# okieraised/rs-face-detection-tflite

Measured on AMD Instinct MI355X. Metric: faces/sec at batch=256 (256x256 back-camera) per GPU, higher is better.
Workload: dtype f32

## Files before the change

rs-face-detection-tflite_amd/csrc/engine.cpp:

```cpp
#include "engine.hpp"
#include "launch.hpp"

#include <algorithm>
#include <cstdio>
#include <cstdlib>
#include <cstring>
#include <stdexcept>

namespace mi {

void hip_check(hipError_t e, const char* what) {
    if (e != hipSuccess) throw std::runtime_error(std::string(what) + ": " + hipGetErrorString(e));
}

namespace {
template <class T>
void upload(T*& dev, std::vector<T>& host, const char* what_alloc, const char* what_copy) {
    if (dev) hip_check(hipFree(dev), "hipFree");
    dev = nullptr;
    if (host.empty()) return;
    hip_check(hipMalloc(reinterpret_cast<void**>(&dev), host.size() * sizeof(T)), what_alloc);
    hip_check(hipMemcpy(dev, host.data(), host.size() * sizeof(T), hipMemcpyHostToDevice), what_copy);
    std::vector<T>().swap(host);
}
// ... 24 lines not shown
    if (d_in_stage_) hipFree(d_in_stage_);
    free_bandnet();
    for (float* p : d_out_)
        if (p) hipFree(p);
    for (hipStream_t st : side_streams_) hipStreamDestroy(st);
    for (hipEvent_t ev : lane_events_) hipEventDestroy(ev);
    for (hipStream_t st : head_streams_) hipStreamDestroy(st);
    for (hipEvent_t ev : head_events_) if (ev) hipEventDestroy(ev);
    if (stream_) hipStreamDestroy(stream_);
}

void Model::invalidate_graphs() {
    if (!graphs_.empty()) (void)hipDeviceSynchronize();
    for (auto& kv : graphs_) hipGraphExecDestroy(kv.second);
    graphs_.clear();
}

struct Model::Option {
    enum { kReplan = 1,
           kFreeSmall = 2,
           kKeepGraphs = 4,
           kOneOf = 8,
           kKiB = 16 , kWriteOnly = 32, kReadOnly = 64,
           kBandGen = 128,
           kForms = 256 };
    const char* key;
    int Model::*field;
    int lo, hi, flags;
};

const Model::Option* Model::find_option(const std::string& key) {
    using O = Option;
    constexpr int kMax = 0x7fffffff;
    static const Option table[] = {
        {"chunk", &Model::chunk_, 0, kMax, 0},
        {"graph", &Model::use_graph_, 0, 1, 0},
        {"fuse", &Model::fuse_level_, 0, 5, O::kReplan},
        {"res_budget", &Model::res_budget_, 16, 156, O::kReplan | O::kKiB},
        {"pipe", &Model::pipe_max_, 0, 4, O::kReplan},
        {"small_chain", &Model::small_chain_, 0, 64, O::kFreeSmall},
        {"pipe_rows", &Model::pipe_rows_, 1 << 1 | 1 << 2 | 1 << 4, 0, O::kOneOf},
        {"pipe_band", &Model::pipe_band_, 0, 4096, 0},
        {"strip", &Model::strip_, 0, 1, 0},
        {"stem_fuse", &Model::stem_fuse_, 0, 1, 0},
        {"stem_mfma", &Model::stem_mfma_, 0, 2, O::kForms},
        {"conv_mfma", &Model::conv_mfma_, 0, 1, 0},
        {"conv_bf16", &Model::conv_bf16_, 0, 2, O::kReplan},
        {"stem_run", &Model::stem_run_, 0, 32, 0},
        {"pair_fuse", &Model::pair_fuse_, 0, 1, 0},
        {"mdb_band", &Model::mdb_band_, 0, 4096, 0},
        {"chain_fixed", &Model::chain_fixed_, 0, 1, 0},
        {"chain_sched", &Model::chain_sched_, 0, 1, 0},
        {"mchain", &Model::mchain_, 0, 1, 0},
        {"tail", &Model::tail_, 0, 1, O::kReplan},
        {"tail_pre", &Model::tail_pre_, 0, 2, 0},
        {"tail_g", &Model::tail_g_, 0, 64, 0},
        {"band", &Model::band_, 0, 2, O::kReplan},
        {"band_test_fail", &Model::band_test_fail_, 0, 1, O::kWriteOnly},
        {"band_test_absent", &Model::band_test_absent_, 0, 256, O::kWriteOnly},
        {"band_test_gen", nullptr, 0, kMax, O::kBandGen | O::kWriteOnly},
        {"band_wide", &Model::band_wide_ok_, 0, 1, O::kReplan},
        {"band_fork", &Model::band_fork_, 0, 1, O::kReplan},
        {"band_nw", &Model::band_nw_, 8, 256, O::kReplan},
        {"band_fail_streak", &Model::band_fail_streak_, 0, 0, O::kReadOnly},
        {"band_wraps", &Model::band_wraps_, 0, 0, O::kReadOnly},
        {"fork", &Model::fork_, 0, 1, 0},
        {"heads", &Model::head_streams_opt_, 1, kHeadStreams, O::kReplan},
        {"reuse", &Model::reuse_, 0, 1, O::kReplan},
        {"lanes", &Model::lanes_, 1, 4, 0},
        {"test_poison", &Model::test_poison_, 1 << 1 | 1 << 2, 0, O::kOneOf | O::kKeepGraphs},
    };
    for (const Option& o : table)
        if (key == o.key) return &o;
    return nullptr;
}

void Model::set_option(const std::string& key, int value) {
    const Option* o = find_option(key);
    if (!o || (o->flags & Option::kReadOnly)) throw std::runtime_error("unknown option '" + key + "'");
    int v = (o->lo == 0 && o->hi == 1) ? value != 0 : std::min(o->hi, std::max(o->lo, value));
    if (o->flags & Option::kOneOf) v = (value >= 0 && value < 31 && (o->lo >> value & 1)) ? value : 0;
    if (o->flags & Option::kForms) v = (value >= o->lo && value <= o->hi) ? value : 1;
    if (o->flags & Option::kKiB) v *= 1024;
    if (o->flags & Option::kBandGen) { band_gen_ = static_cast<unsigned>(v); band_gen_force_ = true; }
    else this->*o->field = v;
    if (o->flags & Option::kKeepGraphs) return;
    if (o->flags & Option::kReplan) dirty_ = true;
    if ((o->flags & Option::kFreeSmall) && d_small_) { hipFree(d_small_); d_small_ = nullptr; small_floats_ = 0; }
    invalidate_graphs();
    chunk_cap_ = 0;
}

int Model::get_option(const std::string& key) const {
    const Option* o = find_option(key);
    if (!o || (o->flags & Option::kWriteOnly)) throw std::runtime_error("unknown option '" + key + "'");
    const int v = this->*o->field;
    return (o->flags & Option::kKiB) ? v / 1024 : v;
}

void Model::rebuild() {
    if (d_small_) { hipFree(d_small_); d_small_ = nullptr; small_floats_ = 0; }
    hip_check(hipSetDevice(device_), "hipSetDevice");
    invalidate_graphs();
    plan_ = build_plan(parse_tflite(blob_.data(), blob_.size()), fuse_level_, pipe_max_, res_budget_, tail_ != 0);
    if (!reuse_) {
        long off = 0;
// ... 137 lines not shown
                const int Cm = g.tensors[m.in[0]].shape[3];
                if (m.kind == Node::Conv) macs += elems(m.out) * m.KH * m.KW * Cm * batch;
                else macs += static_cast<double>(mo[1]) * mo[2] * Cm * ((m.w >= 0 ? 9 : 0) + mo[3]) * batch;
                for (int c : {m.w, m.b, m.w2, m.b2, m.alpha}) bytes += 4 * elems(c);
            }
        }
        if (n.kind == Node::Chain) {
            for (int t : n.extra_out) bytes += 4 * elems(t) * batch;
            for (const Node& m : n.members) {
                const auto& mo = g.tensors[m.out].shape;
                macs += static_cast<double>(mo[1]) * mo[2] * g.tensors[m.in[0]].shape[3] * (9 + mo[3]) * batch;
            }
            for (const Node& m : n.members)
                for (int c : {m.w, m.b, m.w2, m.b2, m.alpha}) bytes += 4 * elems(c);
            for (const Node& m : n.head_nodes) {
                macs += elems(m.out) * g.tensors[m.in[0]].shape[3] * batch;
                for (int c : {m.w, m.b, m.w2, m.b2}) bytes += 4 * elems(c);
            }
        }
        st.bytes += bytes;
        st.macs += macs;
        auto dims = [](const std::vector<int>& sh) {
            std::string d;
            for (size_t q = 1; q < sh.size(); q++) d += (q > 1 ? "x" : "") + std::to_string(sh[q]);
            return d;
        };
        if (static_cast<int>(i) == first.launches[k].node) st.detail = dims(si) + "->";
        st.detail = st.detail.substr(0, st.detail.find("->") + 2) + dims(so);
    }
    return stats;
}

LaunchCtx Model::launch_ctx(const float* in, int chunk_start, int frames) const {
    LaunchCtx c;
    c.weights = d_weights_;
    c.arena = d_arena_ + static_cast<size_t>(plan_.arena_floats_per_frame) * chunk_cap_ * arena_lane_;
    c.in = in; c.out = d_out_.data();
    c.small = d_small_; c.small_floats = small_floats_;
    c.progs = d_programs_; c.tail_progs = d_tail_programs_;
    c.band_prog = d_band_prog_; c.band_consts = d_band_consts_; c.band_ws = d_band_ws_; c.band_sync = d_band_sync_; c.band_fail = d_band_fail_;
    c.chunk_cap = chunk_cap_; c.chunk_start = chunk_start; c.F = frames;
    c.u8_frames = u8_.frames; c.u8_lut = u8_.lut; c.u8_frame_bytes = u8_.frame_bytes; c.u8_row_bytes = u8_.row_bytes;
    c.strip = strip_; c.pair_fuse = pair_fuse_; c.stem_fuse = stem_fuse_; c.stem_mfma = stem_mfma_; c.stem_run = stem_run_; c.mchain = mchain_; c.conv_mfma = conv_mfma_; c.conv_bf16 = conv_bf16_;
    c.small_chain = small_chain_; c.lanes = lanes_;
    c.pipe_rows = pipe_rows_; c.pipe_band = pipe_band_; c.mdb_band = mdb_band_; c.tail_pre = tail_pre_; c.tail_g = tail_g_;
    c.fork = fork_ && lanes_ == 1;
    c.cu_count = device_cu_count();
    c.band = band_use_ && chunk_start == 0;
    c.band_test_absent = band_test_absent_;
    return c;
}

namespace {
int issue(const Launch& l, hipStream_t s, int chain_fixed, int chain_sched) {
    auto many = [&](int (*f)(const BlockArgs*, int, void*)) { return f(l.blocks.data(), static_cast<int>(l.blocks.size()), s); };
    switch (l.to) {
        case Launcher::Conv: return launch_conv(std::get<ConvArgs>(l.args), s);
        case Launcher::HeadGemm: return launch_head_gemm(std::get<HeadGemmArgs>(l.args), s);
        case Launcher::Dw: return launch_dw(std::get<DwArgs>(l.args), s);
        case Launcher::Xc: return launch_xc(std::get<XcArgs>(l.args), s);
        case Launcher::Mdblock: return launch_mdblock(std::get<DblockArgs>(l.args), s);
        case Launcher::Dblock: return launch_dblock(std::get<DblockArgs>(l.args), s);
        case Launcher::Mbneck: return launch_mbneck(std::get<BneckArgs>(l.args), s);
        case Launcher::Bneck: return launch_bneck(std::get<BneckArgs>(l.args), s);
        case Launcher::Tail: return launch_tail(std::get<TailLaunch>(l.args), s);
        case Launcher::Resident: return launch_resident(std::get<ResLaunch>(l.args), s);
        case Launcher::Chain: return launch_chain(std::get<ChainArgs>(l.args), s, chain_fixed, chain_sched);
        case Launcher::StripPipe: return many(launch_strip_pipe);
        case Launcher::MstripChain: return many(launch_mstrip_chain);
        case Launcher::SmallChain: {
            int rc = 0;
            for (size_t k = 0; k < l.blocks.size() && rc == 0; k++) rc = l.blocks[k].sh == 1 ? launch_strip(l.blocks[k], s) : launch_block(l.blocks[k], s);
            return rc;
        }
        case Launcher::Ms2: return launch_ms2(std::get<BlockArgs>(l.args), s);
        case Launcher::Mwalk: return launch_mwalk(std::get<BlockArgs>(l.args), s);
        case Launcher::Strip: return launch_strip(std::get<BlockArgs>(l.args), s);
        case Launcher::Mstrip: return launch_mstrip(std::get<BlockArgs>(l.args), s);
        case Launcher::Block: return launch_block(std::get<BlockArgs>(l.args), s);
        case Launcher::Add: return launch_add(std::get<EltArgs>(l.args), s);
        case Launcher::Act: return launch_act(std::get<EltArgs>(l.args), s);
        case Launcher::Maxpool: return launch_maxpool(std::get<EltArgs>(l.args), s);
        case Launcher::Padc: return launch_padc(std::get<EltArgs>(l.args), s);
        case Launcher::Resize2x: return launch_resize2x(std::get<EltArgs>(l.args), s);
        case Launcher::DepthToSpace: return launch_depth_to_space(std::get<EltArgs>(l.args), s);
        case Launcher::Bandnet: return launch_bandnet(std::get<BandLaunch>(l.args), s);
        case Launcher::Avgpool: return launch_avgpool(std::get<EltArgs>(l.args), s);
        case Launcher::L2norm: return launch_l2norm_rows(std::get<EltArgs>(l.args), s);
        case Launcher::Transpose: return launch_transpose(std::get<EltArgs>(l.args), s);
    }
    return 0;
}
}

void Model::enqueue_chunk(const float* in, int chunk_start, int F, hipStream_t trunk, std::vector<hipEvent_t>* marks, Lowered* keep) {
    LaunchCtx ctx = launch_ctx(in, chunk_start, F);
    if (marks) ctx.fork = false;
    Lowered low = lower_chunk(plan_, consts_, band_plan_, sched_, ctx, keep != nullptr);
    auto mark = [&] {
        if (!marks) return;
        hipEvent_t ev;
        hip_check(hipEventCreate(&ev), "hipEventCreate");
        hip_check(hipEventRecord(ev, trunk), "hipEventRecord");
        marks->push_back(ev);
    };
    mark();
    const size_t n_launches = low.launches.size(), start_event = plan_.nodes.size();
    auto event = [&](size_t k) {
        if (head_events_.size() < plan_.nodes.size() + 2 + kHeadStreams) head_events_.resize(plan_.nodes.size() + 2 + kHeadStreams, nullptr);
        if (!head_events_[k]) hip_check(hipEventCreateWithFlags(&head_events_[k], hipEventDisableTiming), "hipEventCreate");
        return head_events_[k];
    };
    unsigned used_heads = 0;
    for (size_t k = 0; k < n_launches; k++) {
        const Launch& l = low.launches[k];
        hipStream_t s = trunk;
        if (l.slot >= 0) {
            while (static_cast<int>(head_streams_.size()) <= l.slot) {
                hipStream_t st;
                hip_check(hipStreamCreateWithFlags(&st, hipStreamNonBlocking), "hipStreamCreate");
                head_streams_.push_back(st);
            }
            s = head_streams_[static_cast<size_t>(l.slot)];
            if (l.wait >= 0) {
                hip_check(wait_event(s, event(static_cast<size_t>(low.launch_of_node[static_cast<size_t>(l.wait)]))), "hipStreamWaitEvent");
            } else {
                hip_check(record_event(event(start_event), trunk), "hipEventRecord");
                hip_check(wait_event(s, event(start_event)), "hipStreamWaitEvent");
            }
            used_heads |= 1u << l.slot;
        }
        int rc = 0;
        for (int rep = 0; rep < (marks ? profile_inner_ : 1) && rc == 0; rep++) rc = issue(l, s, chain_fixed_, chain_sched_);
        if (rc != 0) throw std::runtime_error(std::string("kernel launch failed: ") + hipGetErrorString(static_cast<hipError_t>(rc)));
        if (l.record) hip_check(record_event(event(k), s), "hipEventRecord");
        mark();
    }
    for (int k = 0; k < kHeadStreams; k++)
        if (used_heads & (1u << k)) {
            hip_check(record_event(event(start_event + 1 + static_cast<size_t>(k)), head_streams_[static_cast<size_t>(k)]), "hipEventRecord");
            hip_check(wait_event(trunk, event(start_event + 1 + static_cast<size_t>(k))), "hipStreamWaitEvent");
        }
    last_chunk_frames_ = F;
    if (keep) *keep = std::move(low);
}

void Model::enqueue_all(const float* in, int batch, hipStream_t s) {
    if (lanes_ > 1 && batch > chunk_cap_) {
        while (static_cast<int>(side_streams_.size()) < lanes_ - 1) {
            hipStream_t st;
            hip_check(hipStreamCreateWithFlags(&st, hipStreamNonBlocking), "hipStreamCreate");
            side_streams_.push_back(st);
        }
        while (static_cast<int>(lane_events_.size()) < lanes_) {
            hipEvent_t ev;
            hip_check(hipEventCreateWithFlags(&ev, hipEventDisableTiming), "hipEventCreate");
            lane_events_.push_back(ev);
        }
        hip_check(record_event(lane_events_[0], s), "hipEventRecord");
        int lane = 0;
        for (int start = 0; start < batch; start += chunk_cap_, lane = (lane + 1) % lanes_) {
            hipStream_t ls = lane == 0 ? s : side_streams_[lane - 1];
            if (lane > 0 && start < chunk_cap_ * lanes_) hip_check(wait_event(ls, lane_events_[0]), "hipStreamWaitEvent");
            arena_lane_ = lane;
            enqueue_chunk(in, start, std::min(chunk_cap_, batch - start), ls);
        }
        arena_lane_ = 0;
        for (int l = 1; l < lanes_; l++) {
            hip_check(record_event(lane_events_[l], side_streams_[l - 1]), "hipEventRecord");
            hip_check(wait_event(s, lane_events_[l]), "hipStreamWaitEvent");
        }
        return;
    }
    int chunk = chunk_cap_;
    for (int start = 0; start < batch; start += chunk) enqueue_chunk(in, start, std::min(chunk, batch - start), s);
}

bool Model::takes_u8_input() {
    if (dirty_) rebuild();
    return mi::takes_u8_input(plan_, consts_);
}

void Model::poison_scratch(hipStream_t s) {
    const int byte = test_poison_ == 1 ? 0xFF : 0x7F;
    if (d_arena_) hip_check(hipMemsetAsync(d_arena_, byte, std::max<size_t>(arena_floats_, 64) * sizeof(float), s), "hipMemsetAsync poison arena");
    if (d_small_) hip_check(hipMemsetAsync(d_small_, byte, small_floats_ * sizeof(float), s), "hipMemsetAsync poison small-batch scratch");
// ... 167 lines not shown
```

rs-face-detection-tflite_amd/csrc/engine.hpp:

```cpp
#pragma once

#include <hip/hip_runtime.h>

#include <map>
#include <memory>
#include <string>
#include <vector>

#include "bandplan.hpp"
#include "consts.hpp"
#include "launches.hpp"
#include "plan.hpp"

namespace mi {

void hip_check(hipError_t e, const char* what);

class Model {
   public:
    Model(const uint8_t* bytes, size_t n, int device);
    ~Model();
    Model(const Model&) = delete;
    Model& operator=(const Model&) = delete;

    int device() const { return device_; }
    const Graph& graph() const { return plan_.graph; }
    const Plan& plan() const { return plan_; }
    std::vector<int> input_dims() const { return plan_.graph.tensors[plan_.graph.inputs[0]].shape; }
    int num_outputs() const { return static_cast<int>(plan_.graph.outputs.size()); }
    const std::vector<int>& output_dims(int i) const { return plan_.graph.tensors[plan_.graph.outputs.at(i)].shape; }
    size_t output_elems(int i) const { return plan_.graph.tensors[plan_.graph.outputs.at(i)].elems(); }
    size_t input_elems() const { return plan_.graph.tensors[plan_.graph.inputs[0]].elems(); }

    void run_device(const float* in, int batch, hipStream_t stream, bool one_shot = false);
    bool band_failed();
    int get_option(const std::string& key) const;
    int band_workgroups(int batch);
    void run(const float* in, int batch, float* const* outs, int mem, hipStream_t stream);
    float* output_device(int i) const { return d_out_.at(i); }
    hipStream_t stream() const { return stream_; }
    bool takes_u8_input();
    void run_device_u8(const uint8_t* frames, long frame_bytes, int row_bytes, const float* lut, int batch, hipStream_t stream);

    struct LaunchStat {
        std::string kernel, detail;
        double ms = 0, bytes = 0, macs = 0;
    };
    std::vector<LaunchStat> profile(const float* in, int batch, int reps, hipStream_t stream);
    void set_option(const std::string& key, int value);
    size_t debug_tensor(int tensor, int frame, float* dst, size_t cap);
    std::string describe() const { return plan_.describe(); }

   private:
    void rebuild();
    struct Option;
    static const Option* find_option(const std::string& key);
    void build_bandnet();
    void free_bandnet();
    bool band_usable(int batch) const;
    void band_before_launch(hipStream_t s);
    void poison_scratch(hipStream_t s);
    void ensure_capacity(int batch);
    LaunchCtx launch_ctx(const float* in, int chunk_start, int frames) const;
    void enqueue_chunk(const float* in, int chunk_start, int frames, hipStream_t s, std::vector<hipEvent_t>* marks = nullptr, Lowered* keep = nullptr);
    void enqueue_all(const float* in, int batch, hipStream_t s);
    void invalidate_graphs();

    int device_ = 0;
    std::vector<uint8_t> blob_;
    Plan plan_;
    int fuse_level_ = 5, pipe_max_ = 4, tail_ = 1, reuse_ = 1;
    int res_budget_ = 156 * 1024;
    int chunk_ = 0, lanes_ = 1, use_graph_ = 1;
    int fork_ = 1, head_streams_opt_ = 1;
    int conv_mfma_ = 1;
    int conv_bf16_ = 0;
    int strip_ = 1, stem_fuse_ = 1, stem_mfma_ = 1, stem_run_ = 0, pair_fuse_ = 1, mchain_ = 1, chain_fixed_ = 1, chain_sched_ = 1;
    int pipe_rows_ = 0, pipe_band_ = 0, mdb_band_ = 0;
    int tail_pre_ = 0, tail_g_ = 0;
    int arena_lane_ = 0;
    std::vector<hipStream_t> side_streams_;
    std::vector<hipEvent_t> lane_events_;
    SideSchedule sched_;
    std::vector<hipStream_t> head_streams_;
    std::vector<hipEvent_t> head_events_;
    bool dirty_ = true;

    float* d_weights_ = nullptr;
    PlanConsts consts_;
    int profile_inner_ = 1;

    ResStage* d_programs_ = nullptr;
    TailStage* d_tail_programs_ = nullptr;
    float* d_arena_ = nullptr;
    size_t arena_floats_ = 0;
    int chunk_cap_ = 0;
    int batch_cap_ = 0;
    std::vector<float*> d_out_;
    float* d_in_stage_ = nullptr;
    size_t in_stage_floats_ = 0;
    int last_chunk_frames_ = 0;

    int band_ = 1;
    int band_nw_ = 128;
    BandPlan band_plan_;
    bool band_use_ = false;
    bool band_ran_ = false;
    int band_test_fail_ = 0;
    int band_test_absent_ = 0;
    int test_poison_ = 0;
    int band_fail_streak_ = 0;
    bool band_disabled_ = false;
    unsigned band_gen_ = 0;
    bool band_gen_force_ = false;
    int band_wraps_ = 0;
    size_t band_ws_bytes_ = 0;
    int band_fork_ = 1, band_wide_ok_ = 1;
    BandPacked* d_band_prog_ = nullptr;
    float* d_band_consts_ = nullptr;
    float* d_band_ws_ = nullptr;
    unsigned* d_band_sync_ = nullptr;
    int* h_band_fail_ = nullptr;
    int* d_band_fail_ = nullptr;

    hipStream_t stream_ = nullptr;
    int small_chain_ = 16;
    float* d_small_ = nullptr;
    size_t small_floats_ = 0;
    struct GraphKey {
        const void* in;
// ... 24 lines not shown
```

rs-face-detection-tflite_amd/csrc/kernels.hpp:

```cpp
#pragma once

#include <cstddef>
#include <cstdint>

namespace mi {

enum ActKind : int { ACT_NONE = 0, ACT_RELU = 1, ACT_RELU6 = 2, ACT_PRELU = 3 };
enum ResMode : int { RES_NONE = 0, RES_DIRECT = 1, RES_MAXPOOL = 2, RES_UP2X = 3 };

struct Epilogue {
    const float* bias = nullptr;
    const float* alpha = nullptr;
    const float* res = nullptr;
    long res_fs = 0;
    int res_mode = RES_NONE;
    int res_C = 0;
    int res_W = 0, res_H = 0;
    int act = ACT_NONE;
    int res_after = 0;
};

struct ConvArgs {
    const float* in = nullptr;
    const uint8_t* in_u8 = nullptr;
// ... 223 lines not shown
    unsigned mHWp = 0, mWp = 0;
    long w_a = -1;
    long w_c = -1;
};
struct TailLaunch {
    const TailStage* prog = nullptr;
    int nstages = 0, B = 0;
    int G = 1;
    int frame_floats = 0;
    int variant = 0;
    ResBases bases;
};
int launch_tail(const TailLaunch& a, void* stream);
bool tail_stage_ok(int kind, int K, int S, int src_C, int Kv, int Co, bool dst_lds);
unsigned tail_magic(int d);

int launch_conv(const ConvArgs& a, void* stream);
const char* conv_kernel_label(const ConvArgs& a);
bool conv_takes_u8(const ConvArgs& a);
bool conv_mfma_shape_ok(int C, int KH, int KW, int Co);
bool conv_mfma_supports(const ConvArgs& a);
int launch_conv_mfma(const ConvArgs& a, void* stream);
bool conv_bf16_supports(const ConvArgs& a);
int launch_conv_bf16(const ConvArgs& a, void* stream);
int launch_dw(const DwArgs& a, void* stream);
int launch_block(const BlockArgs& a, void* stream);
bool block_kernel_supports(const BlockArgs& a);
const char* block_kernel_label(const BlockArgs& a, char* buf, size_t cap);
int launch_strip(const BlockArgs& a, void* stream);
bool strip_kernel_supports(const BlockArgs& a);
bool strip_shape_ok(int C, int Co);
int strip_consts_floats(int C);
void strip_pack_consts(int C, const float* w_dw, const float* b_dw, const float* w_pw, const float* bias, const float* alpha, int act, float* dst);
const char* strip_kernel_label(const BlockArgs& a, char* buf, size_t cap);
int launch_mwalk(const BlockArgs& a, void* stream);
bool mwalk_kernel_supports(const BlockArgs& a);
bool mwalk_shape_ok(int W, int C, int Co);
int mwalk_consts_floats(int W, int C, int Co);
void mwalk_pack_consts(int W, int C, int Co, const float* w_dw, const float* b_dw, const float* w_pw, const float* bias, const float* alpha, int act, float* dst);
const char* mwalk_kernel_label(const BlockArgs& a, char* buf, size_t cap);
int launch_ms2(const BlockArgs& a, void* stream);
bool ms2_kernel_supports(const BlockArgs& a);
bool ms2_shape_ok(int W, int C, int Co, bool skip);
int ms2_consts_floats(int W, int C, int Co, bool skip);
void ms2_pack_consts(int W, int C, int Co, bool skip, const float* w_dw, const float* b_dw, const float* w_pw, const float* bias, const float* alpha, int act, float* dst);
const char* ms2_kernel_label(const BlockArgs& a, char* buf, size_t cap);
int launch_mstrip(const BlockArgs& a, void* stream);
bool mstrip_kernel_supports(const BlockArgs& a);
bool mstrip_shape_ok(int C, int Co);
int mstrip_consts_floats(int C);
void mstrip_pack_consts(int C, const float* w_dw, const float* b_dw, const float* w_pw, const float* bias, const float* alpha, int act, float* dst);
const char* mstrip_kernel_label(const BlockArgs& a, char* buf, size_t cap);
bool mstrip_chain_supports(const BlockArgs* blocks, int n);
int launch_mstrip_chain(const BlockArgs* blocks, int n, void* stream);
bool strip_pipe_supports(const BlockArgs* blocks, int n);
bool strip_pipe_shape_ok(int C, int W);
bool strip_tail_shape_ok(int C, int Co, int H, int W);
int strip_consts_s2_floats(int C, int Co);
void strip_pack_consts_s2(int C, int Co, const float* w_dw, const float* b_dw, const float* w_pw, const float* bias, const float* alpha, int act, float* dst);
int launch_strip_pipe(const BlockArgs* blocks, int n, void* stream);
const char* strip_pipe_label(const BlockArgs* blocks, int n, char* buf, size_t cap);
int strip_pipe_rows_per_step(int H, int hint = 0);
int launch_chain(const ChainArgs& a, void* stream, int fixed = 1, int sched = 1);

struct BneckBlock {
    const float* w1 = nullptr;
    const float* w2 = nullptr;
    const float* consts = nullptr;
    float hi1 = 0.f, hi2 = 0.f;
    const float* mconsts = nullptr;
    int act1 = ACT_RELU, act2 = ACT_RELU;
};
constexpr int kMaxBneck = 6;
struct BneckArgs {
    const float* in = nullptr;
    float* out = nullptr;
    long in_fs = 0, out_fs = 0;
    int B = 0, H = 0, W = 0, C = 0, Cm = 0, nblocks = 0;
    int bands = 1;
    BneckBlock blocks[kMaxBneck];
};
struct XcStage {
    const float* cblob = nullptr;
    int has_dw = 1;
    const float* w_pw = nullptr;
    int C = 0, Co = 0;
    int act = ACT_RELU;
    int skip = 0;
    const float* res = nullptr;
    long res_fs = 0;
    int res_C = 0, res_W = 0;
};
constexpr int kMaxXc = 8;
struct XcArgs {
    const float* in = nullptr;
    float* out = nullptr;
    long in_fs = 0, out_fs = 0;
    int B = 0, H = 0, W = 0, nstages = 0;
    XcStage st[kMaxXc];
};
bool xc_kernel_supports(const XcArgs& a);
int xc_const_floats(int C, int Co);
int launch_xc(const XcArgs& a, void* stream);
struct DblockArgs {
    const float* in = nullptr;
    float* out = nullptr;
    long in_fs = 0, out_fs = 0;
// ... 133 lines not shown
```

rs-face-detection-tflite_amd/csrc/mstrip_kernels.hip:

```cpp
#include <hip/hip_runtime.h>

#include <algorithm>
#include <cstdint>
#include <cstdio>
#include <cstdlib>
#include <type_traits>
#include <utility>

#include "kernels.hpp"
#include "launch.hpp"
#include "mrow.hpp"

namespace mi {

namespace {

struct MstripArgs {
    const float* in;
    float* out;
    const float* consts;
    long in_fs, out_fs;
    int B, H;
    int bands, band_rows;
    int has_res;
    float hi;
    unsigned long long* stamps;
};

constexpr int kMstripChain = 8;
struct MstripChainArgs {
    const float* in[kMstripChain];
    float* out[kMstripChain];
    const float* consts[kMstripChain];
    long in_fs[kMstripChain], out_fs[kMstripChain];
    int has_res[kMstripChain];
    float hi[kMstripChain];
    int nblocks, B, H;
};

template <int CK>
struct MK {
    static constexpr int C = 4 * CK, MT = C / 16;
    static constexpr int QP = CK + 1;
    static constexpr int PS = 4 * QP;
    static constexpr int IMG_F = 34 * PS;
    static constexpr int DPX = 64 / QP;
    static constexpr int NLD = 32 / DPX;
    static_assert(32 % DPX == 0 && NLD == 8, "eight DMA instructions per row (two source bases, four immediate offsets each)");
    static_assert((16 * PS) % 64 == 0 && 16 * PS / 64 < 256, "ds_read2st64_b32 reaches the second pixel tile");
    static constexpr int OFF_A = 0, A_F = CK * MT * 64, OFF_TAP = A_F, TAP_F = CK * 48, OFF_BIAS = OFF_TAP + TAP_F, OFF_SLOPE = OFF_BIAS + C, TOTAL = OFF_SLOPE + C;
    static constexpr int WG_F = A_F + 2 * C + TAP_F;
    static constexpr int NBUF = 2;
};

#ifdef MI_MSTRIP_STAMPS
struct MstripStamps { unsigned long long acc[7] = {0, 0, 0, 0, 0, 0, 0}, prev = __builtin_amdgcn_s_memtime(); };
#define MI_MSTAMP(k) { __builtin_amdgcn_sched_barrier(0); unsigned long long t_ = __builtin_amdgcn_s_memtime(); asm volatile("s_waitcnt lgkmcnt(0)" ::: "memory"); st.acc[k] += t_ - st.prev; st.prev = t_; __builtin_amdgcn_sched_barrier(0); }
#else
struct MstripStamps {};
#define MI_MSTAMP(k)
#endif

template <int CK>
__device__ __forceinline__ void mstrip_issue_row(const float* in, const int r, const int H, const unsigned lds_img, const int bi, const int goff) {
    using K = MK<CK>;
    mrow_dma2<K::C, K::PS, K::DPX, K::DPX * K::QP>(reinterpret_cast<const char*>(in + (long)min(max(r, 0), H - 1) * 32 * K::C),
                                                   lds_img + (unsigned)((bi * K::IMG_F + K::PS) * 4), goff);
}

template <int CK, bool RELU, class HR>
__device__ __forceinline__ void mstrip_walk(const float* in, float* out, const float* wgc, float* img, const unsigned lds_img, const int goff, const HR has_res,
                                            const float hi, const int H, const int y0, const int y1, const int lane, MstripStamps& st) {
    using K = MK<CK>;
    constexpr int C = K::C, MT = K::MT, PS = K::PS, QP = K::QP, IMG_F = K::IMG_F, NLD = K::NLD;
    const int kq = lane >> 4, p = lane & 15;
    float tap[CK][9];
    mrow_load_taps9<CK>(reinterpret_cast<const float4*>(wgc + K::A_F + 2 * C) + kq * 3, tap);
    MI_MSTAMP(0)
    typedef __attribute__((address_space(3))) float lfloat;
    const unsigned x_lds = (unsigned)(uintptr_t)(lfloat*)(img + p * PS + kq);
    const unsigned a_lds = (unsigned)(uintptr_t)(lfloat*)const_cast<float*>(wgc + lane);
    const float* sme = img + (1 + p) * PS + 4 * kq;
    const unsigned ooff = (unsigned)(p * C + 4 * kq) * 4u;

    float accA[CK][2], accB[CK][2];
    df32x4 D[MT][2];
#pragma unroll
    for (int ks = 0; ks < CK; ks++) accA[ks][0] = accA[ks][1] = accB[ks][0] = accB[ks][1] = 0.f;

    constexpr int NST = 2 * MT;
    auto step = [&](auto emit, int r, float (&aPN)[CK][2], float (&aC)[CK][2]) {
        const int t = r - (y0 - 1), bi = t & 1;
        mrow_wait<NST, NLD>(t - 1 >= 2, t == 0 || (t - 1) + 2 <= (y1 - y0 + 1));
        if (r < 0 || r >= H) mrow_clear_row<32 * QP>(img + bi * IMG_F + PS, lane);
        wave_sync();
        MI_MSTAMP(1)
        mstrip_row<CK, MT, PS, decltype(emit)::value>(x_lds + (unsigned)(bi * IMG_F * 4), a_lds, tap, aPN, aC, D);
        MI_MSTAMP(2)
        __builtin_amdgcn_sched_barrier(0);
        if constexpr (decltype(emit)::value) mrow_store_row<RELU, C, 32>(D, (gchar*)(out + (long)(r - 1) * 32 * C), ooff, wgc + K::A_F + C + 4 * kq, hi, p);
        MI_MSTAMP(3)
        __builtin_amdgcn_sched_barrier(0);
        mrow_init_acc<C, PS>(D, wgc + K::A_F + 4 * kq, sme + bi * IMG_F, has_res != 0);
        __builtin_amdgcn_sched_barrier(0);
        wave_sync();
        __builtin_amdgcn_s_waitcnt(0xC07F);
        if (r + 2 <= y1) mstrip_issue_row<CK>(in, r + 2, H, lds_img, bi, goff);
        MI_MSTAMP(4)
    };
    step(std::false_type{}, y0 - 1, accA, accB);
    step(std::false_type{}, y0, accB, accA);
    for (int r = y0 + 1; r <= y1; r += 2) {
        step(std::true_type{}, r, accA, accB);
        if (r + 1 > y1) break;
        step(std::true_type{}, r + 1, accB, accA);
    }
}

template <int CK, bool RELU>
__global__ __launch_bounds__(256, 2) void mstrip_kernel(MstripArgs a) {
    using K = MK<CK>;
    constexpr int C = K::C, PS = K::PS, QP = K::QP, IMG_F = K::IMG_F, NLD = K::NLD, NBUF = K::NBUF;
    extern __shared__ __attribute__((aligned(16))) float lds[];
    MstripStamps st;
    const int lane = threadIdx.x & 63;
    const int wave = __builtin_amdgcn_readfirstlane(threadIdx.x >> 6);
    float* wgc = lds;
    float* img = lds + K::WG_F + wave * NBUF * IMG_F;
    const int unit = blockIdx.x * 4 + wave;
    const int band = unit / a.B, b = unit - band * a.B;
    const bool active = band < a.bands;
    const int y0 = band * a.band_rows, y1 = min(y0 + a.band_rows, a.H);
    const float* in = a.in + (long)b * a.in_fs;
    const int goff = mrow_goff<CK>(lane);
    const unsigned lds_img = __builtin_amdgcn_readfirstlane((unsigned)(uintptr_t)(__attribute__((address_space(3))) float*)img);
    mrow_clear_border<QP, NBUF, IMG_F, 33 * PS>(img, lane);

    if (active) mstrip_issue_row<CK>(in, y0 - 1, a.H, lds_img, 0, goff);
    MI_MSTAMP(5)
    for (int i = threadIdx.x; i < K::A_F / 4; i += 256) reinterpret_cast<float4*>(wgc)[i] = reinterpret_cast<const float4*>(a.consts + K::OFF_A)[i];
    for (int i = threadIdx.x; i < 2 * C; i += 256) wgc[K::A_F + i] = a.consts[K::OFF_BIAS + i];
    for (int i = threadIdx.x; i < K::TAP_F / 4; i += 256) reinterpret_cast<float4*>(wgc + K::A_F + 2 * C)[i] = reinterpret_cast<const float4*>(a.consts + K::OFF_TAP)[i];
    if (active) mstrip_issue_row<CK>(in, y0, a.H, lds_img, 1, goff);
    if (active) wait_vm<NLD>(); else wait_vm<0>();
    MI_MSTAMP(6)
    asm volatile("s_waitcnt lgkmcnt(0)" ::: "memory");
    __builtin_amdgcn_s_barrier();
    asm volatile("" ::: "memory");
    if (!active) return;
    mstrip_walk<CK, RELU>(in, a.out + (long)b * a.out_fs, wgc, img, lds_img, goff, a.has_res != 0, a.hi, a.H, y0, y1, lane, st);
#ifdef MI_MSTRIP_STAMPS
    if (a.stamps && lane == 0)
        for (int k = 0; k < 7; k++) a.stamps[(long)unit * 8 + k] = st.acc[k];
#endif
}

template <int CK, bool RELU>
__global__ __launch_bounds__(512, 2) void mstrip_chain_kernel(MstripChainArgs ca) {
    using K = MK<CK>;
    constexpr int C = K::C, PS = K::PS, QP = K::QP, IMG_F = K::IMG_F, NLD = K::NLD, NBUF = K::NBUF;
    extern __shared__ __attribute__((aligned(16))) float lds[];
    MstripStamps st;
    const int lane = threadIdx.x & 63;
    const int wave = __builtin_amdgcn_readfirstlane(threadIdx.x >> 6);
    float* img = lds + 2 * K::WG_F + wave * NBUF * IMG_F;
    const int b = blockIdx.x;
    const int y0 = 4 * wave, y1 = y0 + 4;
    const int goff = mrow_goff<CK>(lane);
    const unsigned lds_img = __builtin_amdgcn_readfirstlane((unsigned)(uintptr_t)(__attribute__((address_space(3))) float*)img);
    mrow_clear_border<QP, NBUF, IMG_F, 33 * PS>(img, lane);

    for (int i = threadIdx.x; i < K::A_F / 4; i += 512) reinterpret_cast<float4*>(lds)[i] = reinterpret_cast<const float4*>(ca.consts[0] + K::OFF_A)[i];
    for (int i = threadIdx.x; i < 2 * C; i += 512) lds[K::A_F + i] = ca.consts[0][K::OFF_BIAS + i];
    for (int i = threadIdx.x; i < K::TAP_F / 4; i += 512) reinterpret_cast<float4*>(lds + K::A_F + 2 * C)[i] = reinterpret_cast<const float4*>(ca.consts[0] + K::OFF_TAP)[i];
    for (int blk = 0; blk < ca.nblocks; blk++) {
        float* wgc = lds + (blk & 1) * K::WG_F;
        const float* in = ca.in[blk] + (long)b * ca.in_fs[blk];
        const int has_res = ca.has_res[blk];
        const float hi = ca.hi[blk];
        float* const outp = ca.out[blk] + (long)b * ca.out_fs[blk];
        mstrip_issue_row<CK>(in, y0 - 1, ca.H, lds_img, 0, goff);
        constexpr int NPRE = (K::WG_F / 4 + 511) / 512;
        float4 pre[NPRE];
        const bool more = blk + 1 < ca.nblocks;
        if (more) {
            const float* cn = ca.consts[blk + 1];
#pragma unroll
            for (int k = 0; k < NPRE; k++) {
                const int i = threadIdx.x + 512 * k;
                const int src = i < K::A_F / 4 ? K::OFF_A + 4 * i : (i < (K::A_F + 2 * C) / 4 ? K::OFF_BIAS + 4 * i - K::A_F : K::OFF_TAP + 4 * i - K::A_F - 2 * C);
                pre[k] = i < K::WG_F / 4 ? *reinterpret_cast<const float4*>(cn + src) : make_float4(0.f, 0.f, 0.f, 0.f);
            }
        }
        mstrip_issue_row<CK>(in, y0, ca.H, lds_img, 1, goff);
        wait_vm<NLD>();
        asm volatile("s_waitcnt lgkmcnt(0)" ::: "memory");
        if (blk == 0) {
            __builtin_amdgcn_s_barrier();
            asm volatile("" ::: "memory");
        }
        mstrip_walk<CK, RELU>(in, outp, wgc, img, lds_img, goff, has_res, hi, ca.H, y0, y1, lane, st);
        asm volatile("s_waitcnt vmcnt(0)" ::: "memory");
        if (more) {
            float* nx = lds + ((blk + 1) & 1) * K::WG_F;
#pragma unroll
            for (int k = 0; k < NPRE; k++) {
                const int i = threadIdx.x + 512 * k;
                if (i < K::WG_F / 4) reinterpret_cast<float4*>(nx)[i] = pre[k];
            }
        }
        asm volatile("s_waitcnt vmcnt(0) lgkmcnt(0)" ::: "memory");
        __builtin_amdgcn_s_barrier();
        asm volatile("" ::: "memory");
    }
}

}

bool mstrip_shape_ok(int C, int Co) {
    static const bool off = getenv("MI_NO_MSTRIP") != nullptr;
    return !off && C == Co && C == 48;
}

bool mstrip_kernel_supports(const BlockArgs& a) {
    if (!a.w_strip || !a.has_dw || a.sh != 1 || a.sw != 1 || a.pt != 1 || a.pl != 1) return false;
    if (!mstrip_shape_ok(a.C, a.Co) || a.W != 32 || a.H != a.Ho || a.W != a.Wo || a.H < 2) return false;
    if (a.ep.res_mode != RES_NONE) {
        if (a.ep.res_after) return false;
        if (a.ep.res_mode != RES_DIRECT || a.ep.res != a.in || a.ep.res_fs != a.in_fs || a.ep.res_C != a.C) return false;
    }
    static const int min_b = getenv("MI_MSTRIP_MIN_B") ? atoi(getenv("MI_MSTRIP_MIN_B")) : 32;
    if (a.B < min_b) return false;
    auto aligned16 = [](const void* p) { return (reinterpret_cast<uintptr_t>(p) & 15) == 0; };
    return aligned16(a.in) && aligned16(a.out) && !(a.in_fs & 3) && !(a.out_fs & 3);
}

int mstrip_consts_floats(int C) { return C == 48 ? MK<12>::TOTAL : 0; }

void mstrip_pack_consts(int C, const float* w_dw, const float* b_dw, const float* w_pw, const float* bias, const float* alpha, int act, float* dst) {
    using K = MK<12>;
    std::fill(dst, dst + mstrip_consts_floats(C), 0.f);
    mrow_pack_a(dst + K::OFF_A, w_pw, C / 4, K::MT, C);
    mrow_pack_taps(dst + K::OFF_TAP, w_dw, C / 4);
    mrow_pack_bias(dst + K::OFF_BIAS, dst + K::OFF_SLOPE, C, C, w_pw, b_dw, bias, alpha, act);
}

const char* mstrip_kernel_label(const BlockArgs& a, char* buf, size_t cap) {
    snprintf(buf, cap, "mstrip_kernel<%d,%d>", a.C / 4, a.ep.act == ACT_RELU ? 1 : 0);
    return buf;
}

bool mstrip_chain_supports(const BlockArgs* blocks, int n) {
    static const bool off = getenv("MI_NO_MSTRIP_CHAIN") != nullptr;
    if (off || n < 2 || n > kMstripChain) return false;
    for (int k = 0; k < n; k++) {
        const BlockArgs& a = blocks[k];
        if (!mstrip_kernel_supports(a) || a.H != 32 || a.B != blocks[0].B || (a.ep.act == ACT_RELU) != (blocks[0].ep.act == ACT_RELU)) return false;
        if (k && a.in != blocks[k - 1].out) return false;
    }
    return true;
}

int launch_mstrip_chain(const BlockArgs* blocks, int n, void* stream) {
    using K = MK<12>;
    if (!mstrip_chain_supports(blocks, n)) return (int)hipErrorInvalidValue;
    MstripChainArgs ca{};
    ca.nblocks = n; ca.B = blocks[0].B; ca.H = blocks[0].H;
    for (int k = 0; k < n; k++) {
        const BlockArgs& a = blocks[k];
        ca.in[k] = a.in; ca.out[k] = a.out; ca.consts[k] = a.w_strip; ca.in_fs[k] = a.in_fs; ca.out_fs[k] = a.out_fs;
        ca.has_res[k] = a.ep.res_mode == RES_DIRECT;
        ca.hi[k] = a.ep.act == ACT_RELU6 ? 6.f : INFINITY;
    }
    const size_t lds_bytes = (size_t)(2 * K::WG_F + 8 * K::NBUF * K::IMG_F) * 4;
    return mrow_launch(mstrip_chain_kernel<12, true>, mstrip_chain_kernel<12, false>, blocks[0].ep.act == ACT_RELU, dim3((unsigned)ca.B), dim3(512), lds_bytes,
                       (hipStream_t)stream, ca);
}

unsigned long long* g_mstrip_stamps = nullptr;

int launch_mstrip(const BlockArgs& a, void* stream) {
    using K = MK<12>;
    MstripArgs ma;
    ma.stamps = g_mstrip_stamps;
    ma.in = a.in; ma.out = a.out; ma.consts = a.w_strip; ma.in_fs = a.in_fs; ma.out_fs = a.out_fs;
    ma.B = a.B; ma.H = a.H;
    static const int forced = getenv("MI_MSTRIP_BAND") ? atoi(getenv("MI_MSTRIP_BAND")) : 0;
    long bands = std::max<long>(1, (8L * device_cu_count() + a.B / 2) / std::max(1, a.B));
    int rows = (int)((a.H + bands - 1) / bands);
    rows = std::max(rows, std::min(a.H, 4));
    if (forced > 0) rows = std::min(forced, a.H);
    ma.band_rows = rows;
    ma.bands = (a.H + rows - 1) / rows;
    ma.has_res = a.ep.res_mode == RES_DIRECT;
    ma.hi = a.ep.act == ACT_RELU6 ? 6.f : INFINITY;
    const long units = (long)a.B * ma.bands;
    const size_t lds_bytes = (size_t)(K::WG_F + 4 * K::NBUF * K::IMG_F) * 4;
    return mrow_launch(mstrip_kernel<12, true>, mstrip_kernel<12, false>, a.ep.act == ACT_RELU, dim3((unsigned)((units + 3) / 4)), dim3(256), lds_bytes,
                       (hipStream_t)stream, ma);
}

}
```

Measured before the change: 224,700.

## Hand over chained mstrip block boundary rows through LDS instead of refetching

In the multi-block mstrip chain kernel, the last output row of each block is also written into the LDS image buffer, and the next block's first input row is prefetched during the final step. The next block then skips its initial global row fetches and waits. The next block's weights are prefetched with raw asm loads so the vmcnt wait at block end can be dropped. This removes per-block startup latency and global reloads, at the cost of extra barriers and more fragile wait-count reasoning. Optional timestamp instrumentation is added alongside.

```diff
diff --git a/rs-face-detection-tflite_amd/csrc/engine.cpp b/rs-face-detection-tflite_amd/csrc/engine.cpp
--- a/rs-face-detection-tflite_amd/csrc/engine.cpp
+++ b/rs-face-detection-tflite_amd/csrc/engine.cpp
@@ -100,6 +100,7 @@
         {"chain_fixed", &Model::chain_fixed_, 0, 1, 0},
         {"chain_sched", &Model::chain_sched_, 0, 1, 0},
         {"mchain", &Model::mchain_, 0, 1, 0},
+        {"mchain_lds", &Model::mchain_lds_, 0, 1, 0},
         {"tail", &Model::tail_, 0, 1, O::kReplan},
         {"tail_pre", &Model::tail_pre_, 0, 2, 0},
         {"tail_g", &Model::tail_g_, 0, 64, 0},
@@ -343,7 +344,7 @@
 }
 
 namespace {
-int issue(const Launch& l, hipStream_t s, int chain_fixed, int chain_sched) {
+int issue(const Launch& l, hipStream_t s, int chain_fixed, int chain_sched, int mchain_lds) {
     auto many = [&](int (*f)(const BlockArgs*, int, void*)) { return f(l.blocks.data(), static_cast<int>(l.blocks.size()), s); };
     switch (l.to) {
         case Launcher::Conv: return launch_conv(std::get<ConvArgs>(l.args), s);
@@ -358,7 +359,7 @@
         case Launcher::Resident: return launch_resident(std::get<ResLaunch>(l.args), s);
         case Launcher::Chain: return launch_chain(std::get<ChainArgs>(l.args), s, chain_fixed, chain_sched);
         case Launcher::StripPipe: return many(launch_strip_pipe);
-        case Launcher::MstripChain: return many(launch_mstrip_chain);
+        case Launcher::MstripChain: return launch_mstrip_chain(l.blocks.data(), static_cast<int>(l.blocks.size()), s, mchain_lds);
         case Launcher::SmallChain: {
             int rc = 0;
             for (size_t k = 0; k < l.blocks.size() && rc == 0; k++) rc = l.blocks[k].sh == 1 ? launch_strip(l.blocks[k], s) : launch_block(l.blocks[k], s);
@@ -422,7 +423,7 @@
             used_heads |= 1u << l.slot;
         }
         int rc = 0;
-        for (int rep = 0; rep < (marks ? profile_inner_ : 1) && rc == 0; rep++) rc = issue(l, s, chain_fixed_, chain_sched_);
+        for (int rep = 0; rep < (marks ? profile_inner_ : 1) && rc == 0; rep++) rc = issue(l, s, chain_fixed_, chain_sched_, mchain_lds_);
         if (rc != 0) throw std::runtime_error(std::string("kernel launch failed: ") + hipGetErrorString(static_cast<hipError_t>(rc)));
         if (l.record) hip_check(record_event(event(k), s), "hipEventRecord");
         mark();
diff --git a/rs-face-detection-tflite_amd/csrc/engine.hpp b/rs-face-detection-tflite_amd/csrc/engine.hpp
--- a/rs-face-detection-tflite_amd/csrc/engine.hpp
+++ b/rs-face-detection-tflite_amd/csrc/engine.hpp
@@ -75,7 +75,7 @@
     int fork_ = 1, head_streams_opt_ = 1;
     int conv_mfma_ = 1;
     int conv_bf16_ = 0;
-    int strip_ = 1, stem_fuse_ = 1, stem_mfma_ = 1, stem_run_ = 0, pair_fuse_ = 1, mchain_ = 1, chain_fixed_ = 1, chain_sched_ = 1;
+    int strip_ = 1, stem_fuse_ = 1, stem_mfma_ = 1, stem_run_ = 0, pair_fuse_ = 1, mchain_ = 1, mchain_lds_ = 1, chain_fixed_ = 1, chain_sched_ = 1;
     int pipe_rows_ = 0, pipe_band_ = 0, mdb_band_ = 0;
     int tail_pre_ = 0, tail_g_ = 0;
     int arena_lane_ = 0;
diff --git a/rs-face-detection-tflite_amd/csrc/kernels.hpp b/rs-face-detection-tflite_amd/csrc/kernels.hpp
--- a/rs-face-detection-tflite_amd/csrc/kernels.hpp
+++ b/rs-face-detection-tflite_amd/csrc/kernels.hpp
@@ -299,7 +299,7 @@
 void mstrip_pack_consts(int C, const float* w_dw, const float* b_dw, const float* w_pw, const float* bias, const float* alpha, int act, float* dst);
 const char* mstrip_kernel_label(const BlockArgs& a, char* buf, size_t cap);
 bool mstrip_chain_supports(const BlockArgs* blocks, int n);
-int launch_mstrip_chain(const BlockArgs* blocks, int n, void* stream);
+int launch_mstrip_chain(const BlockArgs* blocks, int n, void* stream, int lds_handover = 1);
 bool strip_pipe_supports(const BlockArgs* blocks, int n);
 bool strip_pipe_shape_ok(int C, int W);
 bool strip_tail_shape_ok(int C, int Co, int H, int W);
diff --git a/rs-face-detection-tflite_amd/csrc/mstrip_kernels.hip b/rs-face-detection-tflite_amd/csrc/mstrip_kernels.hip
--- a/rs-face-detection-tflite_amd/csrc/mstrip_kernels.hip
+++ b/rs-face-detection-tflite_amd/csrc/mstrip_kernels.hip
@@ -36,6 +36,9 @@
     int has_res[kMstripChain];
     float hi[kMstripChain];
     int nblocks, B, H;
+#ifdef MI_MSTRIP_STAMPS
+    unsigned long long* stamps;
+#endif
 };
 
 template <int CK>
@@ -53,8 +56,9 @@
     static constexpr int NBUF = 2;
 };
 
-#ifdef MI_MSTRIP_STAMPS
-struct MstripStamps { unsigned long long acc[7] = {0, 0, 0, 0, 0, 0, 0}, prev = __builtin_amdgcn_s_memtime(); };
+constexpr int kMstripStampSlots = 12;
+#ifdef MI_MSTRIP_STAMPS
+struct MstripStamps { unsigned long long acc[kMstripStampSlots] = {0, 0, 0, 0, 0, 0, 0, 0, 0, 0, 0, 0}, prev = __builtin_amdgcn_s_memtime(); };
 #define MI_MSTAMP(k) { __builtin_amdgcn_sched_barrier(0); unsigned long long t_ = __builtin_amdgcn_s_memtime(); asm volatile("s_waitcnt lgkmcnt(0)" ::: "memory"); st.acc[k] += t_ - st.prev; st.prev = t_; __builtin_amdgcn_sched_barrier(0); }
 #else
 struct MstripStamps {};
@@ -68,9 +72,14 @@
                                                    lds_img + (unsigned)((bi * K::IMG_F + K::PS) * 4), goff);
 }
 
-template <int CK, bool RELU, class HR>
+struct MstripHand {
+    bool first, give;
+    const float* next;
+};
+template <int CK, bool RELU, bool HAND = false, class HR>
 __device__ __forceinline__ void mstrip_walk(const float* in, float* out, const float* wgc, float* img, const unsigned lds_img, const int goff, const HR has_res,
-                                            const float hi, const int H, const int y0, const int y1, const int lane, MstripStamps& st) {
+                                            const float hi, const int H, const int y0, const int y1, const int lane, MstripStamps& st,
+                                            const MstripHand hand = MstripHand{true, false, nullptr}) {
     using K = MK<CK>;
     constexpr int C = K::C, MT = K::MT, PS = K::PS, QP = K::QP, IMG_F = K::IMG_F, NLD = K::NLD;
     const int kq = lane >> 4, p = lane & 15;
@@ -91,7 +100,12 @@
     constexpr int NST = 2 * MT;
     auto step = [&](auto emit, int r, float (&aPN)[CK][2], float (&aC)[CK][2]) {
         const int t = r - (y0 - 1), bi = t & 1;
-        mrow_wait<NST, NLD>(t - 1 >= 2, t == 0 || (t - 1) + 2 <= (y1 - y0 + 1));
+        const bool handing = HAND && decltype(emit)::value && hand.next && r == y1;
+        if (handing) {
+            dwg_barrier();
+            MI_MSTAMP(10)
+        }
+        if (!HAND || hand.first || t != 0) mrow_wait<NST, NLD>(t - 1 >= 2, t == 0 || (t - 1) + 2 <= (y1 - y0 + 1));
         if (r < 0 || r >= H) mrow_clear_row<32 * QP>(img + bi * IMG_F + PS, lane);
         wave_sync();
         MI_MSTAMP(1)
@@ -99,6 +113,9 @@
         MI_MSTAMP(2)
         __builtin_amdgcn_sched_barrier(0);
         if constexpr (decltype(emit)::value) mrow_store_row<RELU, C, 32>(D, (gchar*)(out + (long)(r - 1) * 32 * C), ooff, wgc + K::A_F + C + 4 * kq, hi, p);
+        if constexpr (HAND && decltype(emit)::value) {
+            if (handing && hand.give) mrow_store_a<RELU, C, PS>(D, const_cast<float*>(sme) + K::NBUF * IMG_F, wgc + K::A_F + C + 4 * kq, hi, true, kq);
+        }
         MI_MSTAMP(3)
         __builtin_amdgcn_sched_barrier(0);
         mrow_init_acc<C, PS>(D, wgc + K::A_F + 4 * kq, sme + bi * IMG_F, has_res != 0);
@@ -106,6 +123,7 @@
         wave_sync();
         __builtin_amdgcn_s_waitcnt(0xC07F);
         if (r + 2 <= y1) mstrip_issue_row<CK>(in, r + 2, H, lds_img, bi, goff);
+        else if (handing) mstrip_issue_row<CK>(hand.next, y0, H, lds_img, 1, goff);
         MI_MSTAMP(4)
     };
     step(std::false_type{}, y0 - 1, accA, accB);
@@ -155,7 +173,7 @@
 #endif
 }
 
-template <int CK, bool RELU>
+template <int CK, bool RELU, bool LDSH>
 __global__ __launch_bounds__(512, 2) void mstrip_chain_kernel(MstripChainArgs ca) {
     using K = MK<CK>;
     constexpr int C = K::C, PS = K::PS, QP = K::QP, IMG_F = K::IMG_F, NLD = K::NLD, NBUF = K::NBUF;
@@ -179,9 +197,11 @@
         const int has_res = ca.has_res[blk];
         const float hi = ca.hi[blk];
         float* const outp = ca.out[blk] + (long)b * ca.out_fs[blk];
-        mstrip_issue_row<CK>(in, y0 - 1, ca.H, lds_img, 0, goff);
+        const bool fetch = !LDSH || blk == 0;
+        if (fetch) mstrip_issue_row<CK>(in, y0 - 1, ca.H, lds_img, 0, goff);
         constexpr int NPRE = (K::WG_F / 4 + 511) / 512;
         float4 pre[NPRE];
+        df32x4 preh[NPRE];
         const bool more = blk + 1 < ca.nblocks;
         if (more) {
             const float* cn = ca.consts[blk + 1];
@@ -189,30 +209,69 @@
             for (int k = 0; k < NPRE; k++) {
                 const int i = threadIdx.x + 512 * k;
                 const int src = i < K::A_F / 4 ? K::OFF_A + 4 * i : (i < (K::A_F + 2 * C) / 4 ? K::OFF_BIAS + 4 * i - K::A_F : K::OFF_TAP + 4 * i - K::A_F - 2 * C);
-                pre[k] = i < K::WG_F / 4 ? *reinterpret_cast<const float4*>(cn + src) : make_float4(0.f, 0.f, 0.f, 0.f);
+                if constexpr (LDSH) {
+                    const float* gp = cn + (i < K::WG_F / 4 ? src : 0);
+                    asm volatile("global_load_dwordx4 %0, %1, off" : "=v"(preh[k]) : "v"(gp) : "memory");
+                } else {
+                    pre[k] = i < K::WG_F / 4 ? *reinterpret_cast<const float4*>(cn + src) : make_float4(0.f, 0.f, 0.f, 0.f);
+                }
             }
         }
-        mstrip_issue_row<CK>(in, y0, ca.H, lds_img, 1, goff);
-        wait_vm<NLD>();
-        asm volatile("s_waitcnt lgkmcnt(0)" ::: "memory");
+        if (fetch) mstrip_issue_row<CK>(in, y0, ca.H, lds_img, 1, goff);
+        MI_MSTAMP(5)
+        if (fetch) {
+            wait_vm<NLD>();
+            asm volatile("s_waitcnt lgkmcnt(0)" ::: "memory");
+        }
         if (blk == 0) {
             __builtin_amdgcn_s_barrier();
             asm volatile("" ::: "memory");
         }
-        mstrip_walk<CK, RELU>(in, outp, wgc, img, lds_img, goff, has_res, hi, ca.H, y0, y1, lane, st);
-        asm volatile("s_waitcnt vmcnt(0)" ::: "memory");
+        MI_MSTAMP(6)
+        if constexpr (LDSH) {
+            const MstripHand hand{blk == 0, wave < 7, more ? ca.in[blk + 1] + (long)b * ca.in_fs[blk + 1] : nullptr};
+            mstrip_walk<CK, RELU, true>(in, outp, wgc, img, lds_img, goff, has_res, hi, ca.H, y0, y1, lane, st, hand);
+        } else {
+            mstrip_walk<CK, RELU>(in, outp, wgc, img, lds_img, goff, has_res, hi, ca.H, y0, y1, lane, st);
+            asm volatile("s_waitcnt vmcnt(0)" ::: "memory");
+        }
+        MI_MSTAMP(7)
         if (more) {
             float* nx = lds + ((blk + 1) & 1) * K::WG_F;
 #pragma unroll
             for (int k = 0; k < NPRE; k++) {
                 const int i = threadIdx.x + 512 * k;
-                if (i < K::WG_F / 4) reinterpret_cast<float4*>(nx)[i] = pre[k];
+                if constexpr (LDSH) {
+                    asm volatile("" : "+v"(preh[k]));
+                    if (i < K::WG_F / 4) reinterpret_cast<df32x4*>(nx)[i] = preh[k];
+                } else {
+                    if (i < K::WG_F / 4) reinterpret_cast<float4*>(nx)[i] = pre[k];
+                }
             }
         }
-        asm volatile("s_waitcnt vmcnt(0) lgkmcnt(0)" ::: "memory");
+        if constexpr (LDSH) asm volatile("s_waitcnt lgkmcnt(0)" ::: "memory");
+        else asm volatile("s_waitcnt vmcnt(0) lgkmcnt(0)" ::: "memory");
+        MI_MSTAMP(8)
         __builtin_amdgcn_s_barrier();
         asm volatile("" ::: "memory");
-    }
+        MI_MSTAMP(9)
+#ifdef MI_MSTRIP_STAMPS
+        {
+            unsigned long long* park = reinterpret_cast<unsigned long long*>(lds + 2 * K::WG_F + 8 * NBUF * IMG_F) + (wave * kMstripChain + blk) * kMstripStampSlots;
+            for (int k = 0; k < kMstripStampSlots; k++) {
+                if (lane == 0) park[k] = st.acc[k];
+                st.acc[k] = 0;
+            }
+        }
+#endif
+    }
+#ifdef MI_MSTRIP_STAMPS
+    if (ca.stamps) {
+        const unsigned long long* park = reinterpret_cast<const unsigned long long*>(lds + 2 * K::WG_F + 8 * NBUF * IMG_F) + wave * kMstripChain * kMstripStampSlots;
+        asm volatile("s_waitcnt lgkmcnt(0)" ::: "memory");
+        for (int i = lane; i < ca.nblocks * kMstripStampSlots; i += 64) ca.stamps[((long)b * 8 + wave) * kMstripChain * kMstripStampSlots + i] = park[i];
+    }
+#endif
 }
 
 }
@@ -261,7 +320,9 @@
     return true;
 }
 
-int launch_mstrip_chain(const BlockArgs* blocks, int n, void* stream) {
+unsigned long long* g_mstrip_stamps = nullptr;
+
+int launch_mstrip_chain(const BlockArgs* blocks, int n, void* stream, int lds_handover) {
     using K = MK<12>;
     if (!mstrip_chain_supports(blocks, n)) return (int)hipErrorInvalidValue;
     MstripChainArgs ca{};
@@ -272,12 +333,16 @@
         ca.has_res[k] = a.ep.res_mode == RES_DIRECT;
         ca.hi[k] = a.ep.act == ACT_RELU6 ? 6.f : INFINITY;
     }
-    const size_t lds_bytes = (size_t)(2 * K::WG_F + 8 * K::NBUF * K::IMG_F) * 4;
-    return mrow_launch(mstrip_chain_kernel<12, true>, mstrip_chain_kernel<12, false>, blocks[0].ep.act == ACT_RELU, dim3((unsigned)ca.B), dim3(512), lds_bytes,
-                       (hipStream_t)stream, ca);
-}
-
-unsigned long long* g_mstrip_stamps = nullptr;
+    size_t lds_bytes = (size_t)(2 * K::WG_F + 8 * K::NBUF * K::IMG_F) * 4;
+#ifdef MI_MSTRIP_STAMPS
+    ca.stamps = g_mstrip_stamps;
+    lds_bytes += (size_t)8 * kMstripChain * kMstripStampSlots * 8;
+#endif
+    const bool relu = blocks[0].ep.act == ACT_RELU;
+    if (lds_handover)
+        return mrow_launch(mstrip_chain_kernel<12, true, true>, mstrip_chain_kernel<12, false, true>, relu, dim3((unsigned)ca.B), dim3(512), lds_bytes, (hipStream_t)stream, ca);
+    return mrow_launch(mstrip_chain_kernel<12, true, false>, mstrip_chain_kernel<12, false, false>, relu, dim3((unsigned)ca.B), dim3(512), lds_bytes, (hipStream_t)stream, ca);
+}
 
 int launch_mstrip(const BlockArgs& a, void* stream) {
     using K = MK<12>;
```

New measurement: 226,300, median of 6. About the same (+0.7%).
